# SimonMacLean/NeRF-or-nothing

Measured on AMD Instinct MI355X. Metric: train rays/sec (128 samples/ray, 8×256 MLP) at 1/2/4/8 MI355X; PSNR vs ref, higher is better.
Workload: dtype f32; 1 GPU; BASELINE configs[1]: 1024-ray global batch x 128+128 samples, 8x256 MLP fwd/bwd + Adam; global_batch=1024, rays_per_gpu=1024, micro_batch=1024, parallelism=dp1, precision=f32

## Files before the change

nerf-or-nothing_amd/csrc/host/accelerated.cpp:

```cpp
#include "accelerated.h"

#include <algorithm>
#include <cmath>
#include <cstring>

#include "../kernels/common.h"
#include "../kernels/mlp_common.h"
#include "../kernels/mlp_h32.h"
#include "trace.h"

namespace AcceleratedNeRFUtils {

using nof::kBlk;

void KernelTimer::enable(uint32_t mask, hipStream_t st) {
  mask_ = mask;
  st_ = st;
  used_ = 0;
  recs_.clear();
  for (int i = 0; i < NOF_NUM_TIMERS; ++i) { tot_ms_[i] = 0.0f; tot_n_[i] = 0; }
}
void KernelTimer::fold() {
  if (!recs_.empty()) NOF_HIP(hipEventSynchronize(recs_.back().b));
  for (const Rec& r : recs_) {
// ... 553 lines not shown
  }
  if ((size_t)so > slab_cap_ || items.size() * 256 > bias_slabs_.n) {
    NOF_HIP(hipStreamSynchronize(st_));
    slab_cap_ = std::max((size_t)so, slab_cap_);
    slabs_.alloc(slab_cap_);
    bias_slabs_.alloc(std::max(items.size() * 256, bias_slabs_.n));
  }
  std::vector<nof::WgOut> outs;
  int max_elems = 0;
  for (const OutSpec& s : os) {
    nof::WgOut o;
    o.item0 = first_item[s.prob];
    o.nitems = 0;
    NOF_REQUIRE(nlev <= nof::kWgMaxLevels, "too many levels");
    o.nlev = nlev;
    for (int l = 0; l < nlev; ++l) {
      NOF_REQUIRE(first_item[s.prob + l] == o.item0 + o.nitems, "a problem's items are not contiguous");
      o.lev_items[l] = nitems[s.prob + l];
      o.nitems += nitems[s.prob + l];
    }
    o.row_off = s.row_off; o.nrows = s.nrows; o.col_off = s.col_off; o.ncols = s.ncols;
    o.dst = s.dst; o.ld = s.ld; o.dst_col = s.dst_col; o.bias_dst = s.bias; o.prob = s.prob;
    outs.push_back(o);
    max_elems = std::max(max_elems, nof::wgrad_reduce_threads(s.nrows, s.ncols, s.col_off));
  }
  Schedule& sc = sched_[key];
  sc.probs.alloc(P.size());
  sc.items.alloc(items.size());
  sc.item_ptr.alloc(item_ptr.size());
  sc.slab_off.alloc(slab_off.size());
  sc.outs.alloc(outs.size());
  NOF_HIP(hipMemcpy(sc.probs.p, P.data(), P.size() * sizeof(P[0]), hipMemcpyHostToDevice));
  NOF_HIP(hipMemcpy(sc.items.p, items.data(), items.size() * sizeof(items[0]), hipMemcpyHostToDevice));
  NOF_HIP(hipMemcpy(sc.item_ptr.p, item_ptr.data(), item_ptr.size() * sizeof(int), hipMemcpyHostToDevice));
  NOF_HIP(hipMemcpy(sc.slab_off.p, slab_off.data(), slab_off.size() * sizeof(int64_t), hipMemcpyHostToDevice));
  NOF_HIP(hipMemcpy(sc.outs.p, outs.data(), outs.size() * sizeof(outs[0]), hipMemcpyHostToDevice));
  sc.nouts = (int)outs.size();
  sc.max_elems = max_elems;
  sc.num_wg = nwg;
  sc.lv0 = lv0;
  return sc;
}

void AcceleratedMLP::run_wgrad(Schedule& sc, int accumulate) {
  tb(kTWgrad);
  if (precision_ != NOF_PRECISION_F32)
    NOF_HIP(nof::launch_wgrad_x3(sc.probs.p, sc.items.p, sc.item_ptr.p, sc.num_wg, sc.slab_off.p, slabs_.p,
                                 bias_slabs_.p, precision_, st_));
  else
    NOF_HIP(nof::launch_wgrad(sc.probs.p, sc.items.p, sc.item_ptr.p, sc.num_wg, sc.slab_off.p, slabs_.p,
                              bias_slabs_.p, st_));
  te(kTWgrad);
  tb(kTWgradReduce);
  NOF_HIP(nof::launch_wgrad_reduce(sc.outs.p, sc.nouts, sc.max_elems, sc.items.p, sc.probs.p, sc.slab_off.p,
                                   slabs_.p, bias_slabs_.p, accumulate,
                                   f16_pieces() ? amax_.p + sc.lv0 : nullptr, st_));
  te(kTWgradReduce);
}

nof::BwdArgs AcceleratedMLP::bwd_args(int level, const float* color_grad, const float* density_grad) {
  Level& L = lv_[level];
  nof::BwdArgs b{};
  b.M = L.M;
  b.split = precision_;
  b.dbias = cfg_.density_bias;
  b.rgb_scale = rgb_scale();
  if (f16_pieces()) {
    if ((amax_given_ >> level) & 1u) {
      amax_given_ &= ~(1u << level);
    } else {
      const bool cleared = (amax_cleared_ >> level) & 1u;
      amax_cleared_ &= ~(1u << level);
      NOF_HIP(nof::launch_delta_amax(density_grad, color_grad, L.M, amax_.p + level, st_, numeric_.p, cleared));
    }
    b.amax = amax_.p + level;
  }
  b.dsigma = density_grad; b.drgb = color_grad; b.zhead = L.zhead.p;
  b.masks = L.masks.p;
  b.wimg_b = wimg_b_.p;
  b.delta = L.delta.p; b.delta9x = L.delta9x.p;
  return b;
}

void AcceleratedMLP::run_backward(int level, const float* color_grad, const float* density_grad) {
  const nof::BwdArgs b = bwd_args(level, color_grad, density_grad);
  tb(kTMlpBwd);
  NOF_HIP(nof::launch_mlp_bwd(b, st_));
  te(kTMlpBwd);
}

void AcceleratedMLP::run_backward2(int level, const float* const* color_grads, const float* const* density_grads) {
  nof::BwdArgs b = bwd_args(level, color_grads[0], density_grads[0]);
  const nof::BwdArgs b1 = bwd_args(level + 1, color_grads[1], density_grads[1]);
  b.M1 = b1.M; b.dsigma1 = b1.dsigma; b.drgb1 = b1.drgb; b.zhead1 = b1.zhead; b.amax1 = b1.amax;
  b.masks1 = b1.masks; b.delta1 = b1.delta; b.delta9x1 = b1.delta9x;
  tb(kTMlpBwd);
  NOF_HIP(nof::launch_mlp_bwd(b, st_));
  te(kTMlpBwd);
}

float* const* AcceleratedMLP::wgrad_levels(int lv0, int lv1, int accumulate, bool buckets) {
  if (!buckets) {
    run_wgrad(schedule(lv0, lv1), accumulate);
  } else {
    for (int bk = 0; bk < kBuckets; ++bk) {
      run_wgrad(schedule(lv0, lv1, bk), accumulate);
      int64_t off[2], cnt[2];
      const int ns = bucket_spans(bk, off, cnt);
      TraceRange hr("nof:gradient_bucket_hook");
      hook_(hook_user_, bk, ns, off, cnt);
    }
  }
  return grad_views_.data();
}

float* const* AcceleratedMLP::get_gradient(const float* color_grad, const float* density_grad, int level,
                                           uint32_t flags) {
  NOF_REQUIRE(level >= 0 && level < (int)lv_.size(), "level out of range");
  Level& L = lv_[level];
  NOF_REQUIRE(L.M > 0, "get_gradient before get_output for this level");
  NOF_REQUIRE(color_grad && density_grad, "null output gradients");
  NOF_REQUIRE((flags & ~(uint32_t)(NOF_GRAD_ACCUMULATE | NOF_GRAD_PUBLISH)) == 0, "unknown gradient flags");
  const bool buckets = (flags & NOF_GRAD_PUBLISH) && hook_;
  if (generic_) {
    gen_backward(level, color_grad, density_grad, (level > 0 || (flags & NOF_GRAD_ACCUMULATE)) ? 1 : 0);
    return gen_publish(buckets);
  }
  if (!buckets) (void)schedule(level, level + 1);
  else
    for (int b = 0; b < kBuckets; ++b) (void)schedule(level, level + 1, b);
  run_backward(level, color_grad, density_grad);
  return wgrad_levels(level, level + 1, (level > 0 || (flags & NOF_GRAD_ACCUMULATE)) ? 1 : 0, buckets);
}

float* const* AcceleratedMLP::get_gradient_levels(const float* const* color_grads, const float* const* density_grads,
                                                  uint32_t flags) {
  const int nl = (int)lv_.size();
  NOF_REQUIRE(color_grads && density_grads, "null output gradients");
  for (int l = 0; l < nl; ++l) {
    NOF_REQUIRE(lv_[l].M > 0, "get_gradient before get_output for a level");
    NOF_REQUIRE(color_grads[l] && density_grads[l], "null output gradients");
  }
  NOF_REQUIRE((flags & ~(uint32_t)(NOF_GRAD_ACCUMULATE | NOF_GRAD_PUBLISH)) == 0, "unknown gradient flags");
  const bool buckets = (flags & NOF_GRAD_PUBLISH) && hook_;
  if (generic_) {
    for (int l = 0; l < nl; ++l)
      gen_backward(l, color_grads[l], density_grads[l], (l > 0 || (flags & NOF_GRAD_ACCUMULATE)) ? 1 : 0);
    return gen_publish(buckets);
  }
  if (!buckets) (void)schedule(0, nl);
  else
    for (int b = 0; b < kBuckets; ++b) (void)schedule(0, nl, b);
  int l = 0;
  if (precision_ == NOF_PRECISION_F16)
    for (; l + 1 < nl; l += 2) run_backward2(l, color_grads + l, density_grads + l);
  for (; l < nl; ++l) run_backward(l, color_grads[l], density_grads[l]);
  return wgrad_levels(0, nl, (flags & NOF_GRAD_ACCUMULATE) ? 1 : 0, buckets);
}

static nof::GemmSrc gsrc(const float* p, int64_t si, int64_t sk, int idiv = 1) {
  nof::GemmSrc s;
  s.p = p; s.si = si; s.sk = sk; s.idiv = idiv;
  return s;
}

bool AcceleratedMLP::gen_product(nof::GemmArgs a, int ksplit, bool ws, bool f32) {
  int v;
  if (ksplit == 1) {
    a.kchunk = (a.K1 + a.K2 + 15) / 16 * 16;
    a.slab_stride = 0;
  }
  if (ws && !f16_products() && (!a.G || a.mask_in)) {
    nof::GemmArgs w = a;
    w.G = nullptr;
    if (nof::gemm_ws_fits(w)) {
      NOF_HIP(nof::launch_gemm_ws(w, st_, &v));
      tally(v);
      return true;
    }
  }
  NOF_REQUIRE(a.G || !a.mask_in, "a ReLU-bit mask needs the weight-stationary kernel");
  a.mask_in = nullptr;
  a.mask_out = nullptr;
  if (f16_products() && !f32) {
    NOF_HIP(nof::launch_gemm_h(a, ksplit, st_, &v));
    tally_h(v);
  } else {
    NOF_HIP(nof::launch_gemm(a, ksplit, st_, &v));
    tally(v);
  }
  return false;
}

void AcceleratedMLP::gen_split(int nout, int ncols, int M, int* ksplit, int* kchunk) {
  const int tiles = ((nout + 63) / 64) * ((ncols + 63) / 64);
  int ks = std::max(1, std::min((1024 + tiles - 1) / tiles, M / 64));
  const int kc = ((M + ks - 1) / ks + 15) / 16 * 16;
  *kchunk = kc;
  *ksplit = (M + kc - 1) / kc;
}

void AcceleratedMLP::gen_alloc() {
  const int NL = cfg_.num_levels;
  lv_.resize(NL);
  gl_.resize(NL);
  for (int l = 0; l < NL; ++l) {
    Level& L = lv_[l];
    GenLevel& G = gl_[l];
    L.cap = cfg_.max_rays * cfg_.num_samples[l];
    const size_t M = L.cap;
    G.mean.alloc(3 * M); G.cov.alloc(3 * M);
    G.enc_pos.alloc(M * gP_);
    G.enc_dir.alloc((size_t)cfg_.max_rays * gVd_);
    G.h.alloc((size_t)gD_ * M * gW_);
    G.hc.alloc((size_t)gDc_ * M * gWc_);
    G.z.alloc(4 * M);
    G.mbits.alloc((size_t)(gD_ + gDc_) * M * 4);
    G.mb_ok.assign(gD_ + gDc_, 0);
    L.sigma.alloc(M);
    L.rgb.alloc(3 * M);
    max_M_ = std::max(max_M_, L.cap);
  }
  const size_t Wm = std::max(gW_, gWc_);
  gd0_.alloc((size_t)max_M_ * Wm);
  gd1_.alloc((size_t)max_M_ * Wm);
  gdz_.alloc((size_t)max_M_ * 4);
  gray_.alloc((size_t)cfg_.max_rays * gWc_);
  if (cross_) denc_alloc(1);
  if (f16_products()) {
    amax_.alloc(NL);
    NOF_HIP(hipMemset(amax_.p, 0, NL * sizeof(uint32_t)));
  }
  size_t slab = 0;
  for (int l = 0; l < NL; ++l) {
    Level& L = lv_[l];
    size_t need = 0;
    wg_need_ = &need;
    L.M = L.cap; L.n = cfg_.max_rays; L.S = cfg_.num_samples[l];
    gen_backward(l, nullptr, nullptr, 0);
    L.M = L.n = L.S = 0;
    slab = std::max(slab, need);
  }
  wg_need_ = nullptr;
  gslab_.alloc(std::max<size_t>(slab, 1));
}

void AcceleratedMLP::denc_alloc(int first_level) {
  size_t Mx = 0;
  for (int l = first_level; l < (int)lv_.size(); ++l) Mx = std::max(Mx, (size_t)lv_[l].cap);
  int contrib = 1;
  for (int l = 1; l < gD_; ++l) contrib += l % gskip_ == 0 ? 1 : 0;
  const size_t parts = contrib > 2 ? (size_t)((contrib + 1) / 2) : 0;
  if (gd2_.n >= Mx * gW_ && gdenc_.n >= Mx * gP_ && gdenc_part_.n >= parts * Mx * gP_) return;
  if (gd2_.p) NOF_HIP(hipStreamSynchronize(st_));
  gd2_.alloc(Mx * gW_);
  gdenc_.alloc(Mx * gP_);
  if (parts) gdenc_part_.alloc(parts * Mx * gP_);
}

void AcceleratedMLP::set_ray_grad(bool on) {
  if (on) {
    if (!generic_)
      throw Error(NOF_ERR_UNSUPPORTED,
                  "ray gradients need the any-shape path: the fused 8x256 kernels produce no gradient of the encoded "
                  "input (use NOF_PRECISION_F16_PRODUCTS, or NOF_PRECISION_F32 with stop_level_grad = 0)");
    denc_alloc(0);
    if (!gddir_.p) {
      gddir_.alloc((size_t)cfg_.max_rays * gVd_);
      rg_o_.alloc(3 * (size_t)cfg_.max_rays);
      rg_d_.alloc(3 * (size_t)cfg_.max_rays);
    }
  }
  ray_grad_ = on;
  rg_job_ = RayGradJob();
}

void AcceleratedMLP::gen_wgrad(float* dst, int64_t ld, const float* dz, int64_t ldz, int nout, nof::GemmSrc x,
                               int ncols, int M, int accumulate, float* bias_dst, const uint32_t* scale) {
  int ks, kc;
  gen_split(nout, ncols, M, &ks, &kc);
  const size_t need = (size_t)ks * nout * (ncols + 1);
  if (wg_need_) {
    *wg_need_ += need;
    return;
  }
  NOF_REQUIRE(wg_off_ + need <= gslab_.n, "split-K slabs too small");
  float* slab = gslab_.p + wg_off_;
  wg_off_ += need;
  nof::GemmArgs a;
  a.M = nout; a.N = ncols; a.K1 = M;
  a.A1 = gsrc(dz, 1, ldz);
  a.B1 = x;
  a.C = slab; a.ci = ncols; a.cj = 1;
  a.kchunk = kc; a.slab_stride = (int64_t)nout * ncols;
  float* bias_part = slab + (size_t)ks * nout * ncols;
  if (bias_dst) a.rowsum = bias_part;
  if (scale) { a.scale_amax = scale; a.scale_src = 1; }
  gen_product(a, ks, false, !scale);
  wg_jobs_.push_back({slab, dst, a.slab_stride, ld, nout, ncols, ncols, ks, accumulate});
  if (bias_dst) wg_jobs_.push_back({bias_part, bias_dst, nout, nout, 1, nout, nout, ks, accumulate});
}

void AcceleratedMLP::gen_forward(int level, const float* ep, const float* ed) {
  Level& L = lv_[level];
  GenLevel& G = gl_[level];
  const int M = L.M, S = L.S, D = gD_, W = gW_, Dc = gDc_, Wc = gWc_, P = gP_, Vd = gVd_, lr = D + 1 + Dc;
  G.ep = ep; G.ed = ed;
// ... 668 lines not shown
```

nerf-or-nothing_amd/csrc/kernels/mlp16.h:

```cpp
#pragma once
#include "mlp_common.h"

namespace nof {

constexpr int kMlp16Threads = 512;
constexpr int kIpe16Floats = 6 * 64 * 4;

__device__ __forceinline__ f32x4 mfma16(float a, float b, f32x4 c) {
  return __builtin_amdgcn_mfma_f32_16x16x4f32(a, b, c, 0, 0, 0);
}

__device__ __forceinline__ void slice16_dma_step(const float* __restrict__ src, float* dst, int tid, int i) {
  const int wave = tid >> 6;
  const __amdgpu_buffer_rsrc_t rsrc =
      __builtin_amdgcn_make_buffer_rsrc(const_cast<float*>(src), (short)0, 0x7fffffff, 0x00020000);
  __builtin_amdgcn_raw_ptr_buffer_load_lds(rsrc, (lptr_t)(dst + (kMlp16Threads * i + 64 * wave) * 4), 16, tid * 16,
                                           i * kMlp16Threads * 16, 0, 0);
}
__device__ __forceinline__ void slice16_dma(const float* __restrict__ src, float* dst, int tid) {
#pragma unroll
  for (int i = 0; i < 4; ++i) slice16_dma_step(src, dst, tid, i);
}

template <int P> constexpr int ring16_slots() { return P == 0 ? 4 : 3; }
template <int P> constexpr int ring16_floats() { return ring16_slots<P>() * kSliceFloats; }
__device__ __forceinline__ void ring16_prologue(const float* __restrict__ img, float* lds, int tid) {
  slice16_dma(img, lds, tid);
  slice16_dma(img + kSliceFloats, lds + kSliceFloats, tid);
}

__device__ __forceinline__ constexpr int feat16(int t, int g, int r) { return 16 * t + 4 * g + r; }

constexpr int kStoreNT = 2;
struct BlkStore16 {
  static constexpr bool kHalf = false;
  uint32_t voff[4];
  __device__ __forceinline__ BlkStore16(int lane, int half) {
    const int g = lane >> 4, s = 16 * half + (lane & 15);
#pragma unroll
    for (int r = 0; r < 4; ++r)
      voff[r] = 512u * g + ((((s >> 2) ^ (4 * (g & 1) + r)) << 4) | ((s & 3) << 2));
  }
  __device__ __forceinline__ void store(__amdgpu_buffer_rsrc_t blk, int t, int r, float v) const {
    __builtin_amdgcn_raw_buffer_store_b32(__float_as_uint(v), blk, (int)voff[r], 2048 * t + 128 * r, kStoreNT);
  }
};
__device__ __forceinline__ __amdgpu_buffer_rsrc_t blk_rsrc(float* blk) {
  return __builtin_amdgcn_make_buffer_rsrc(blk, (short)0, 0x7fffffff, 0x00020000);
}

template <bool kNT>
struct BlkStore16H {
  static constexpr bool kHalf = true;
  uint32_t voff;
  uint32_t voff2;
  uint32_t sel;
  __device__ __forceinline__ BlkStore16H(int lane, int half) {
    const int g = lane >> 4, j = lane & 15;
    voff = 256u * g + ((((2 * half + (j >> 3)) ^ g) << 4) | ((j & 7) << 1));
    voff2 = 256u * g + 64u * (j & 1) + ((((2 * half + (j >> 3)) ^ g) << 4) | ((j & 6) << 1));
    sel = (j & 1) ? 0x03020706u : 0x05040100u;
  }
  __device__ __forceinline__ void store_pairs(__amdgpu_buffer_rsrc_t blk, int t, uint32_t p01, uint32_t p23) const {
    const uint32_t q01 = (uint32_t)__builtin_amdgcn_mov_dpp((int)p01, 0xB1, 0xF, 0xF, false);
    const uint32_t q23 = (uint32_t)__builtin_amdgcn_mov_dpp((int)p23, 0xB1, 0xF, 0xF, false);
    __builtin_amdgcn_raw_buffer_store_b32(__builtin_amdgcn_perm(q01, p01, sel), blk, (int)voff2, 1024 * t,
                                          kNT ? kStoreNT : 0);
    __builtin_amdgcn_raw_buffer_store_b32(__builtin_amdgcn_perm(q23, p23, sel), blk, (int)voff2 + 128, 1024 * t,
                                          kNT ? kStoreNT : 0);
  }
  __device__ __forceinline__ void store(__amdgpu_buffer_rsrc_t blk, int t, int r, float v) const {
    store_h(blk, t, r, (_Float16)v);
  }
  __device__ __forceinline__ void store_h(__amdgpu_buffer_rsrc_t blk, int t, int r, _Float16 h) const {
    __builtin_amdgcn_raw_buffer_store_b16(__builtin_bit_cast(unsigned short, h), blk, (int)voff + 64 * r, 1024 * t,
                                          kNT ? kStoreNT : 0);
  }
};
template <int P, bool kBwd> struct Store16 { typedef BlkStore16 T; typedef float E; };
template <bool kBwd> struct Store16<2, kBwd> { typedef BlkStore16H<true> T; typedef _Float16 E; };
template <class E>
__device__ __forceinline__ __amdgpu_buffer_rsrc_t blk_rsrc_t(E* blk) {
  return __builtin_amdgcn_make_buffer_rsrc(blk, (short)0, 0x7fffffff, 0x00020000);
}

__device__ __forceinline__ uint2* mask16_ptr(uint32_t* masks, int blk, int slot, int half, int lane) {
  return reinterpret_cast<uint2*>(mask_ptr(masks, blk, slot) + half * 128) + lane;
}
__device__ __forceinline__ bool mask16_bit(const uint2& m, int t, int r) {
  return ((t >> 3 ? m.y : m.x) >> (31 - ((t & 7) * 4 + r))) & 1u;
}
__device__ __forceinline__ float mask16_apply(const uint2& m, int t, int r, float v) {
  const uint32_t w = t >> 3 ? m.y : m.x;
  uint32_t all;
  asm("v_bfe_i32 %0, %1, %2, 1" : "=v"(all) : "v"(w), "n"(31 - ((t & 7) * 4 + r)));
  return __uint_as_float(__float_as_uint(v) & all);
}

__device__ __forceinline__ float relu_bit(float z, uint32_t& mw) {
  const int h = max(__float_as_int(z), 0);
  asm volatile("v_cmp_lt_i32 vcc, 0, %1\n\tv_addc_co_u32 %0, vcc, %0, %0, vcc" : "+v"(mw) : "v"(h) : "vcc");
  return __int_as_float(h);
}

__device__ __forceinline__ void split4h(const float (&x)[4], uint32_t& hi01, uint32_t& hi23, uint32_t& lo01,
                                        uint32_t& lo23) {
  typedef _Float16 h2 __attribute__((ext_vector_type(2)));
  typedef float f2 __attribute__((ext_vector_type(2)));
  hi01 = __builtin_bit_cast(uint32_t, __builtin_convertvector((f2{x[0], x[1]}), h2));
  hi23 = __builtin_bit_cast(uint32_t, __builtin_convertvector((f2{x[2], x[3]}), h2));
  float r[4];
  asm("v_fma_mix_f32 %0, %1, 1.0, -%2 op_sel_hi:[0,0,1]" : "=v"(r[0]) : "v"(x[0]), "v"(hi01));
  asm("v_fma_mix_f32 %0, %1, 1.0, -%2 op_sel:[0,0,1] op_sel_hi:[0,0,1]" : "=v"(r[1]) : "v"(x[1]), "v"(hi01));
  asm("v_fma_mix_f32 %0, %1, 1.0, -%2 op_sel_hi:[0,0,1]" : "=v"(r[2]) : "v"(x[2]), "v"(hi23));
  asm("v_fma_mix_f32 %0, %1, 1.0, -%2 op_sel:[0,0,1] op_sel_hi:[0,0,1]" : "=v"(r[3]) : "v"(x[3]), "v"(hi23));
  lo01 = __builtin_bit_cast(uint32_t, __builtin_convertvector((f2{r[0], r[1]}), h2));
  lo23 = __builtin_bit_cast(uint32_t, __builtin_convertvector((f2{r[2], r[3]}), h2));
}

template <bool kSplit, bool kStore, class ST>
__device__ __forceinline__ void put_tile(float (&bin)[16][4], int t, const float (&v)[4], const ST& bst,
                                         __amdgpu_buffer_rsrc_t blk) {
  if constexpr (kSplit) {
    uint32_t hi01, hi23, lo01, lo23;
    split4h(v, hi01, hi23, lo01, lo23);
    const int row = t & ~1, c = 2 * (t & 1);
    bin[row][c] = __uint_as_float(hi01);
    bin[row][c + 1] = __uint_as_float(hi23);
    bin[row + 1][c] = __uint_as_float(lo01);
    bin[row + 1][c + 1] = __uint_as_float(lo23);
    if constexpr (kStore) {
      if constexpr (ST::kHalf) {
        bst.store_pairs(blk, t, hi01, hi23);
      } else {
#pragma unroll
        for (int r = 0; r < 4; ++r) bst.store(blk, t, r, v[r]);
      }
    }
  } else {
#pragma unroll
    for (int r = 0; r < 4; ++r) {
      bin[t][r] = v[r];
      if constexpr (kStore) bst.store(blk, t, r, v[r]);
    }
  }
}

struct NoEpi16 {
  static constexpr int kVmPerPart = 0;
  __device__ __forceinline__ void operator()(int) {}
};

template <int NT_B, int NT_I, int OT, int kSlots, class Epi>
__device__ __forceinline__ void mlp_layer16(const float (&bin)[16][4], const float* ipe, f32x4 (&acc)[16],
                                            float* lds, int& cur, const float*& wsrc, bool last_in_schedule, int tid,
                                            int lane, Epi& epi, const float* cinit) {
  static_assert(OT % 2 == 0 && OT <= 16, "row tiles come in pairs");
  constexpr int NG = OT;
  constexpr int kEpiGroup1 = 4;
  constexpr int kEpiGroup2 = (NG / 2 + 4 < NG) ? NG / 2 + 4 : NG - 1;
  const int g = lane >> 4;
  const int row = lane & 15;
  const int swz = (row >> 1) & 7;
#pragma unroll
  for (int t = 0; t < NT_B + NT_I; ++t) {
    const bool dma = !(last_in_schedule && t + 2 >= NT_B + NT_I);
    const int nxt2 = kSlots == 4 ? ((cur + 2) & 3) : (cur == 0 ? 2 : cur - 1);
    const float* W = lds + cur * kSliceFloats + row * 32;
    auto aread = [&](int q, int which) {
      const int tt = q / (OT / 2), p = q % (OT / 2);
      return *reinterpret_cast<const f32x4*>(W + (2 * p + which) * 16 * 32 + (((4 * tt + g) ^ swz) << 2));
    };
    f32x4 a0 = aread(0, 0), a1 = aread(0, 1);
    auto cread = [&](int p, int which) { return *reinterpret_cast<const f32x4*>(cinit + 16 * (2 * p + which)); };
    f32x4 c0 = {}, c1 = {};
    if (t == 0 && cinit) { c0 = cread(0, 0); c1 = cread(0, 1); }
#pragma unroll
    for (int q = 0; q < NG; ++q) {
      const int tt = q / (OT / 2), p = q % (OT / 2);
      f32x4 b4;
      if (t < NT_B) {
        const int tb = (t < NT_B) ? 2 * t + tt : 0;
        b4[0] = bin[tb][0]; b4[1] = bin[tb][1]; b4[2] = bin[tb][2]; b4[3] = bin[tb][3];
      } else {
        const int ti = (t >= NT_B) ? 2 * (t - NT_B) + tt : 0;
        if constexpr (kSlots == 4) {
          b4[0] = ipe[4 * ti]; b4[1] = ipe[4 * ti + 1]; b4[2] = ipe[4 * ti + 2]; b4[3] = ipe[4 * ti + 3];
        } else b4 = *reinterpret_cast<const f32x4*>(ipe + (ti * 64 + lane) * 4);
      }
      asm volatile("" ::"v"(a0), "v"(a1), "v"(c0), "v"(c1));
      f32x4 n0 = a0, n1 = a1, m0 = c0, m1 = c1;
      if (q + 1 < NG) {
        n0 = aread(q + 1, 0);
        n1 = aread(q + 1, 1);
      }
      if (t == 0 && cinit && q + 1 < OT / 2) { m0 = cread(q + 1, 0); m1 = cread(q + 1, 1); }
      if (dma && q < 4) slice16_dma_step(wsrc + 2 * kSliceFloats, lds + nxt2 * kSliceFloats, tid, q);
      __builtin_amdgcn_sched_barrier(0);
      const bool first = t == 0 && tt == 0;
#pragma unroll
      for (int r = 0; r < 4; ++r) {
        acc[2 * p] = mfma16(a0[r], b4[r], (first && r == 0) ? c0 : acc[2 * p]);
        acc[2 * p + 1] = mfma16(a1[r], b4[r], (first && r == 0) ? c1 : acc[2 * p + 1]);
      }
      if (t + 1 < NT_B && q == kEpiGroup1) epi(2 * t + 2);
      if (t + 1 < NT_B && q == kEpiGroup2) epi(2 * t + 3);
      __builtin_amdgcn_sched_barrier(0);
      a0 = n0;
      a1 = n1;
      c0 = m0;
      c1 = m1;
    }
    if constexpr (kSlots == 4) {
      if (cur & 1) slice_barrier(t + 1 < NT_B ? 2 * Epi::kVmPerPart : 0);
      cur = (cur + 1) & 3;
    } else {
      slice_barrier((dma ? 4 : 0) + (t + 1 < NT_B ? 2 * Epi::kVmPerPart : 0));
      cur = cur == 2 ? 0 : cur + 1;
    }
    wsrc += kSliceFloats;
  }
}
template <int NT_B, int NT_I, int OT, class Epi>
__device__ __forceinline__ void mlp_layer16h(const float (&bin)[16][4], const float* ipe_lds, f32x4 (&acc)[16],
                                             float* lds, int& cur, const float*& wsrc, bool last_in_schedule, int tid,
                                             int lane, Epi& epi, const float* cinit) {
  typedef SplitMode<2> SM;
  static_assert(OT % 2 == 0 && OT <= 16, "row tiles come in pairs");
  constexpr int kPieces = 2;
  constexpr int kPP0 = 0;
  constexpr int kDmaSteps = 4;
  constexpr int kSlots = ring16_slots<2>();
  constexpr int NG = OT / 2;
  constexpr int kE1 = NG > 4 ? 4 : NG - 1;
  constexpr int kE2 = NG > 6 ? 6 : NG - 1;
#pragma unroll
  for (int t = 0; t < NT_B + NT_I; ++t) {
    const bool dma = !(last_in_schedule && t + 2 >= NT_B + NT_I);
    const int nxt2 = kSlots == 4 ? ((cur + 2) & 3) : (cur == 0 ? 2 : cur - 1);
    const f16x8* W = reinterpret_cast<const f16x8*>(lds + cur * kSliceFloats) + lane;
    Frag<2> b;
    float v[8];
    if (t < NT_B) {
      const int tb = t < NT_B ? 2 * t : 0;
      const f32x4 hi = {bin[tb][0], bin[tb][1], bin[tb][2], bin[tb][3]};
      const f32x4 lo = {bin[tb + 1][0], bin[tb + 1][1], bin[tb + 1][2], bin[tb + 1][3]};
      b.p[0] = __builtin_bit_cast(f16x8, hi);
      b.p[1] = __builtin_bit_cast(f16x8, lo);
    } else {
      const int ti = t >= NT_B ? 2 * (t - NT_B) : 0;
      if constexpr (kSlots == 4) {
#pragma unroll
        for (int i = 0; i < 8; ++i) v[i] = ipe_lds[4 * ti + i];
      } else {
        const f32x4 u0 = *reinterpret_cast<const f32x4*>(ipe_lds + (ti * 64 + lane) * 4);
        const f32x4 u1 = *reinterpret_cast<const f32x4*>(ipe_lds + ((ti + 1) * 64 + lane) * 4);
#pragma unroll
        for (int i = 0; i < 4; ++i) { v[i] = u0[i]; v[4 + i] = u1[i]; }
      }
      split8<2>(v, b);
    }
    Frag<2> a0, a1;
#pragma unroll
    for (int p = 0; p < kPieces; ++p) { a0.p[p] = W[(16 * p) * 64]; a1.p[p] = W[(16 * p + 1) * 64]; }
    auto cread = [&](int rt) { return *reinterpret_cast<const f32x4*>(cinit + 16 * rt); };
    f32x4 c0 = {}, c1 = {};
    if (t == 0 && cinit) { c0 = cread(0); c1 = cread(1); }
#pragma unroll
    for (int q = 0; q < NG; ++q) {
      if constexpr (kPieces == 2) asm volatile("" ::"v"(a0.p[0]), "v"(a0.p[1]), "v"(a1.p[0]), "v"(a1.p[1]), "v"(c0), "v"(c1));
      else asm volatile("" ::"v"(a0.p[0]), "v"(a1.p[0]), "v"(c0), "v"(c1));
      Frag<2> n0 = a0, n1 = a1;
      f32x4 m0 = c0, m1 = c1;
      if (t == 0 && cinit && q + 1 < NG) { m0 = cread(2 * q + 2); m1 = cread(2 * q + 3); }
      if (q + 1 < NG) {
#pragma unroll
        for (int p = 0; p < kPieces; ++p) {
          n0.p[p] = W[(16 * p + 2 * q + 2) * 64];
          n1.p[p] = W[(16 * p + 2 * q + 3) * 64];
        }
      }
      if (dma && q < kDmaSteps) slice16_dma_step(wsrc + 2 * kSliceFloats, lds + nxt2 * kSliceFloats, tid, q);
      __builtin_amdgcn_sched_barrier(0);
      const bool first = t == 0;
#pragma unroll
      for (int pp = kPP0; pp < SM::NPROD; ++pp) {
        acc[2 * q] = SM::mfma16(a0.p[SM::pa(pp)], b.p[SM::pb(pp)], (first && pp == kPP0) ? c0 : acc[2 * q]);
        acc[2 * q + 1] = SM::mfma16(a1.p[SM::pa(pp)], b.p[SM::pb(pp)], (first && pp == kPP0) ? c1 : acc[2 * q + 1]);
      }
      if (t + 1 < NT_B && q == kE1) epi(2 * t + 2);
      if (t + 1 < NT_B && q == kE2) epi(2 * t + 3);
      __builtin_amdgcn_sched_barrier(0);
      a0 = n0;
      a1 = n1;
      c0 = m0;
      c1 = m1;
    }
    if constexpr (kSlots == 4) {
      if (cur & 1) slice_barrier(t + 1 < NT_B ? 2 * Epi::kVmPerPart : 0);
      cur = (cur + 1) & 3;
    } else {
      slice_barrier((dma ? kDmaSteps : 0) + (t + 1 < NT_B ? 2 * Epi::kVmPerPart : 0));
      cur = cur == 2 ? 0 : cur + 1;
    }
    wsrc += kSliceFloats;
  }
}

template <int P, int NT_B, int NT_I, int OT, class Epi>
__device__ __forceinline__ void layer16(const float (&bin)[16][4], const float* ipe_lds, f32x4 (&acc)[16], float* lds,
                                        int& cur, const float*& wsrc, bool last_in_schedule, int tid, int lane,
                                        Epi& epi, const float* cinit = nullptr) {
  if constexpr (P == 2 || P == 3)
    mlp_layer16h<NT_B, NT_I, OT>(bin, ipe_lds, acc, lds, cur, wsrc, last_in_schedule, tid, lane, epi, cinit);
  else
    mlp_layer16<NT_B, NT_I, OT, ring16_slots<P>()>(bin, ipe_lds, acc, lds, cur, wsrc, last_in_schedule, tid, lane,
                                                   epi, cinit);
}
template <int P, int NT_B, int NT_I, int OT>
__device__ __forceinline__ void layer16(const float (&bin)[16][4], const float* ipe_lds, f32x4 (&acc)[16], float* lds,
                                        int& cur, const float*& wsrc, bool last_in_schedule, int tid, int lane,
                                        const float* cinit = nullptr) {
  NoEpi16 none;
  layer16<P, NT_B, NT_I, OT>(bin, ipe_lds, acc, lds, cur, wsrc, last_in_schedule, tid, lane, none, cinit);
}

}
```

nerf-or-nothing_amd/csrc/kernels/mlp_bwd16.hip:

```cpp
#include "common.h"
#include "launch.h"
#include "mlp16.h"

namespace nof {


template <bool kDensity, class ST, bool kSplit = false>
struct BwdEpi16 {
  static constexpr int kVmPerPart = 4;
  const f32x4 (&acc)[16];
  float (&bin)[16][4];
  const ST& bst;
  const int g;
  const float* w8;
  float dzs;
  __amdgpu_buffer_rsrc_t dst_blk;
  uint2 mk;
  f32x4 wnext;

  __device__ __forceinline__ BwdEpi16(const f32x4 (&acc_)[16], float (&bin_)[16][4], const ST& bst_, int lane)
      : acc(acc_), bin(bin_), bst(bst_), g(lane >> 4) {}
  template <class E>
  __device__ __forceinline__ void begin(const uint2* mask, E* dst_blk_, const float* w8_ = nullptr, float dzs_ = 0.0f) {
    mk = *mask;
    dst_blk = blk_rsrc_t(dst_blk_);
    if constexpr (kDensity) {
      w8 = w8_ + 4 * g;
      dzs = dzs_;
      wnext = *reinterpret_cast<const f32x4*>(w8);
    }
  }
  __device__ __forceinline__ void operator()(int t) {
    f32x4 w4;
    if constexpr (kDensity) {
      w4 = wnext;
      if (t + 1 < 16) wnext = *reinterpret_cast<const f32x4*>(w8 + 16 * (t + 1));
    }
    float v[4];
#pragma unroll
    for (int r = 0; r < 4; ++r) {
      v[r] = acc[t][r];
      if constexpr (kDensity) v[r] = __builtin_fmaf(w4[r], dzs, v[r]);
      v[r] = mask16_apply(mk, t, r, v[r]);
    }
    put_tile<kSplit, true>(bin, t, v, bst, dst_blk);
  }
  __device__ __forceinline__ void tile01() {
    (*this)(0);
    (*this)(1);
  }
};

template <int P>
__global__ __launch_bounds__(kMlp16Threads, 1) void k_mlp_bwd16(BwdArgs a) {
  typedef typename Store16<P, true>::T ST;
  typedef typename Store16<P, true>::E AE;
  __shared__ __attribute__((aligned(16))) float lds[ring16_floats<P>() + 256];
  float* w8_lds = lds + ring16_floats<P>();
  const int tid = threadIdx.x, lane = tid & 63, g = lane >> 4, j = lane & 15;
  const int wave = __builtin_amdgcn_readfirstlane(tid >> 6);
  const int half = wave & 1;
  const ST bst(lane, half);
  const int nblk = a.M / kBlk;
  const int blk_raw = blockIdx.x * 4 + (wave >> 1);
  const int blk = blk_raw < nblk ? blk_raw : nblk - 1;
  const int m = blk * kBlk + 16 * half + j;
  NOF_DCHECK(a.M % kBlk == 0 && blk >= 0 && blk < nblk, kChkMlpBlock);
  const float* tail = a.wimg_b + (size_t)kBwdSlices * kSliceFloats;
  const size_t layer_stride = (size_t)nblk * kWidth * kBlk;
  uint32_t* masks = const_cast<uint32_t*>(a.masks);

  ring16_prologue(a.wimg_b, lds, tid);

  const f32x4 zh = reinterpret_cast<const f32x4*>(a.zhead)[m];
  float dzs = a.dsigma[m] * sigmoid_f(zh[0] + a.dbias);
  float dzc[3];
#pragma unroll
  for (int c = 0; c < 3; ++c) {
    const float s = sigmoid_f(zh[1 + c]);
    dzc[c] = a.drgb[(size_t)m * 3 + c] * (s * (1.0f - s)) * a.rgb_scale;
  }
  if constexpr (P >= 2) {
    const float sc = delta_scale(a.amax, false);
    dzs *= sc;
#pragma unroll
    for (int c = 0; c < 3; ++c) dzc[c] *= sc;
  }
  const __amdgpu_buffer_rsrc_t d9 = blk_rsrc_t(reinterpret_cast<AE*>(a.delta9x) + (size_t)blk * kD9F * kBlk);
#pragma unroll
  for (int r = 0; r < 4; ++r) bst.store(d9, 8, r, g == 0 ? (r == 0 ? dzs : dzc[r - 1]) : 0.0f);
  float bin[16][4];
  {
    const uint2 mk = *mask16_ptr(masks, blk, 8, half, lane);
    const float* w10 = tail + kBwdTailW10;
#pragma unroll
    for (int t = 0; t < 8; ++t) {
      const int fb = 16 * t + 4 * g;
      const f32x4 wa = *reinterpret_cast<const f32x4*>(w10 + fb);
      const f32x4 wb = *reinterpret_cast<const f32x4*>(w10 + 128 + fb);
      const f32x4 wc = *reinterpret_cast<const f32x4*>(w10 + 256 + fb);
      float v[4];
#pragma unroll
      for (int r = 0; r < 4; ++r)
        v[r] = mask16_apply(mk, t, r, __builtin_fmaf(wc[r], dzc[2], __builtin_fmaf(wb[r], dzc[1], wa[r] * dzc[0])));
      put_tile<P >= 2, true>(bin, t, v, bst, d9);
    }
  }
  if (tid < 64) reinterpret_cast<f32x4*>(w8_lds)[tid] = reinterpret_cast<const f32x4*>(tail + kBwdTailW8)[tid];
  __syncthreads();

  int cur = 0;
  const float* wsrc = a.wimg_b;
  f32x4 accA[16], accB[16];
  AE* delta_blk = reinterpret_cast<AE*>(a.delta) + (size_t)blk * kWidth * kBlk;
  BwdEpi16<true, ST, P >= 2> e7(accA, bin, bst, lane);
  e7.begin(mask16_ptr(masks, blk, 7, half, lane), delta_blk + 7 * layer_stride, w8_lds, dzs);
  layer16<P, 4, 0, 16>(bin, nullptr, accA, lds, cur, wsrc, false, tid, lane);
  e7.tile01();
  BwdEpi16<false, ST, P >= 2> ea(accA, bin, bst, lane), eb(accB, bin, bst, lane);
  eb.begin(mask16_ptr(masks, blk, 6, half, lane), delta_blk + 6 * layer_stride);
  layer16<P, 8, 0, 16>(bin, nullptr, accB, lds, cur, wsrc, false, tid, lane, e7);
  eb.tile01();
  static_assert(kDepth == 8, "bwd pairing assumes 8 trunk layers");
  for (int l = kDepth - 2; l >= 2; l -= 2) {
    ea.begin(mask16_ptr(masks, blk, l - 1, half, lane), delta_blk + (l - 1) * layer_stride);
    layer16<P, 8, 0, 16>(bin, nullptr, accA, lds, cur, wsrc, false, tid, lane, eb);
    ea.tile01();
    eb.begin(mask16_ptr(masks, blk, l - 2, half, lane), delta_blk + (l - 2) * layer_stride);
    layer16<P, 8, 0, 16>(bin, nullptr, accB, lds, cur, wsrc, l == 2, tid, lane, ea);
    eb.tile01();
  }
#pragma unroll
  for (int t = 2; t < 16; ++t) eb(t);
}

hipError_t launch_mlp_bwd16(const BwdArgs& a, hipStream_t st) {
  const int nblk = a.M / kBlk;
  if (a.split == 2) hipLaunchKernelGGL(k_mlp_bwd16<2>, dim3((nblk + 3) / 4), dim3(kMlp16Threads), 0, st, a);
  else if (a.split == 3) hipLaunchKernelGGL(k_mlp_bwd16<3>, dim3((nblk + 3) / 4), dim3(kMlp16Threads), 0, st, a);
  else hipLaunchKernelGGL(k_mlp_bwd16<0>, dim3((nblk + 3) / 4), dim3(kMlp16Threads), 0, st, a);
  return hipGetLastError();
}

NOF_CHECK_UNIT(check_unit_mlp_bwd16)

}
```

Before: 163,700 rays/s.

## Make f32 MLP backward a persistent kernel spanning both levels with prefetch

The f32 backward MLP kernel becomes persistent: the grid is capped at the CU count and each block loops over block-groups from both levels, coarse and fine. While the last layer of the current group runs, it DMAs the next group's per-ray inputs and the first weight slices into LDS, which hides prologue latency and launch overhead. W10 and W8 are staged in LDS once per block. The host now uses the paired run_backward2 path for F32 too. In exchange the kernel uses more LDS and inline asm LDS reads, and it relies on the run_backward2 path setting M1 and the second-level pointers correctly.

```diff
diff --git a/nerf-or-nothing_amd/csrc/host/accelerated.cpp b/nerf-or-nothing_amd/csrc/host/accelerated.cpp
--- a/nerf-or-nothing_amd/csrc/host/accelerated.cpp
+++ b/nerf-or-nothing_amd/csrc/host/accelerated.cpp
@@ -729,7 +729,7 @@
   else
     for (int b = 0; b < kBuckets; ++b) (void)schedule(0, nl, b);
   int l = 0;
-  if (precision_ == NOF_PRECISION_F16)
+  if (precision_ == NOF_PRECISION_F16 || precision_ == NOF_PRECISION_F32)
     for (; l + 1 < nl; l += 2) run_backward2(l, color_grads + l, density_grads + l);
   for (; l < nl; ++l) run_backward(l, color_grads[l], density_grads[l]);
   return wgrad_levels(0, nl, (flags & NOF_GRAD_ACCUMULATE) ? 1 : 0, buckets);
diff --git a/nerf-or-nothing_amd/csrc/kernels/mlp16.h b/nerf-or-nothing_amd/csrc/kernels/mlp16.h
--- a/nerf-or-nothing_amd/csrc/kernels/mlp16.h
+++ b/nerf-or-nothing_amd/csrc/kernels/mlp16.h
@@ -154,7 +154,7 @@
 template <int NT_B, int NT_I, int OT, int kSlots, class Epi>
 __device__ __forceinline__ void mlp_layer16(const float (&bin)[16][4], const float* ipe, f32x4 (&acc)[16],
                                             float* lds, int& cur, const float*& wsrc, bool last_in_schedule, int tid,
-                                            int lane, Epi& epi, const float* cinit) {
+                                            int lane, Epi& epi, const float* cinit, const float* wrap_src) {
   static_assert(OT % 2 == 0 && OT <= 16, "row tiles come in pairs");
   constexpr int NG = OT;
   constexpr int kEpiGroup1 = 4;
@@ -164,7 +164,10 @@
   const int swz = (row >> 1) & 7;
 #pragma unroll
   for (int t = 0; t < NT_B + NT_I; ++t) {
-    const bool dma = !(last_in_schedule && t + 2 >= NT_B + NT_I);
+    const bool past = last_in_schedule && t + 2 >= NT_B + NT_I;
+    const float* src2 = !past ? wsrc + 2 * kSliceFloats
+                              : (wrap_src ? wrap_src + (t + 2 - (NT_B + NT_I)) * kSliceFloats : nullptr);
+    const bool dma = src2 != nullptr;
     const int nxt2 = kSlots == 4 ? ((cur + 2) & 3) : (cur == 0 ? 2 : cur - 1);
     const float* W = lds + cur * kSliceFloats + row * 32;
     auto aread = [&](int q, int which) {
@@ -195,7 +198,7 @@
         n1 = aread(q + 1, 1);
       }
       if (t == 0 && cinit && q + 1 < OT / 2) { m0 = cread(q + 1, 0); m1 = cread(q + 1, 1); }
-      if (dma && q < 4) slice16_dma_step(wsrc + 2 * kSliceFloats, lds + nxt2 * kSliceFloats, tid, q);
+      if (dma && q < 4) slice16_dma_step(src2, lds + nxt2 * kSliceFloats, tid, q);
       __builtin_amdgcn_sched_barrier(0);
       const bool first = t == 0 && tt == 0;
 #pragma unroll
@@ -310,12 +313,12 @@
 template <int P, int NT_B, int NT_I, int OT, class Epi>
 __device__ __forceinline__ void layer16(const float (&bin)[16][4], const float* ipe_lds, f32x4 (&acc)[16], float* lds,
                                         int& cur, const float*& wsrc, bool last_in_schedule, int tid, int lane,
-                                        Epi& epi, const float* cinit = nullptr) {
+                                        Epi& epi, const float* cinit = nullptr, const float* wrap_src = nullptr) {
   if constexpr (P == 2 || P == 3)
     mlp_layer16h<NT_B, NT_I, OT>(bin, ipe_lds, acc, lds, cur, wsrc, last_in_schedule, tid, lane, epi, cinit);
   else
     mlp_layer16<NT_B, NT_I, OT, ring16_slots<P>()>(bin, ipe_lds, acc, lds, cur, wsrc, last_in_schedule, tid, lane,
-                                                   epi, cinit);
+                                                   epi, cinit, wrap_src);
 }
 template <int P, int NT_B, int NT_I, int OT>
 __device__ __forceinline__ void layer16(const float (&bin)[16][4], const float* ipe_lds, f32x4 (&acc)[16], float* lds,
diff --git a/nerf-or-nothing_amd/csrc/kernels/mlp_bwd16.hip b/nerf-or-nothing_amd/csrc/kernels/mlp_bwd16.hip
--- a/nerf-or-nothing_amd/csrc/kernels/mlp_bwd16.hip
+++ b/nerf-or-nothing_amd/csrc/kernels/mlp_bwd16.hip
@@ -1,3 +1,5 @@
+#include <algorithm>
+
 #include "common.h"
 #include "launch.h"
 #include "mlp16.h"
@@ -51,34 +53,134 @@
   }
 };
 
+__device__ __forceinline__ uint32_t lane_id_opaque() {
+  uint32_t id;
+  asm volatile("v_mbcnt_lo_u32_b32 %0, -1, 0\n\tv_mbcnt_hi_u32_b32 %0, -1, %0" : "=v"(id));
+  return id;
+}
+__device__ __forceinline__ int opaque_vgpr(int v) {
+  asm volatile("" : "+v"(v));
+  return v;
+}
+__device__ __forceinline__ void bwd16_read_inputs(uint32_t base, uint32_t lane, uint32_t j, uint2& mk, f32x4& zh,
+                                                  float (&dr)[3], float& ds) {
+  typedef uint32_t u32x2 __attribute__((ext_vector_type(2)));
+  u32x2 mkv;
+  asm volatile(
+      "ds_read_b64 %0, %6\n\tds_read_b128 %1, %7 offset:512\n\tds_read_b32 %2, %8 offset:768\n\t"
+      "ds_read_b32 %3, %8 offset:772\n\tds_read_b32 %4, %8 offset:776\n\tds_read_b32 %5, %9 offset:960\n\t"
+      "s_waitcnt lgkmcnt(0)"
+      : "=&v"(mkv), "=&v"(zh), "=&v"(dr[0]), "=&v"(dr[1]), "=&v"(dr[2]), "=&v"(ds)
+      : "v"(base + 8u * lane), "v"(base + 16u * j), "v"(base + 12u * j), "v"(base + 4u * j)
+      : "memory");
+  mk = {mkv[0], mkv[1]};
+}
+__device__ __forceinline__ void lds_dma16(const void* p, float* dst, uint32_t voff) {
+  __builtin_amdgcn_raw_ptr_buffer_load_lds(
+      __builtin_amdgcn_make_buffer_rsrc(const_cast<void*>(p), (short)0, 0x7fffffff, 0x00020000), (lptr_t)dst, 16,
+      voff, 0, 0, 0);
+}
+__device__ __forceinline__ void lds_dma4(const void* p, float* dst, uint32_t voff) {
+  __builtin_amdgcn_raw_ptr_buffer_load_lds(
+      __builtin_amdgcn_make_buffer_rsrc(const_cast<void*>(p), (short)0, 0x7fffffff, 0x00020000), (lptr_t)dst, 4,
+      voff, 0, 0, 0);
+}
+__device__ __forceinline__ uint32_t lds_addr(const float* p) {
+  return (uint32_t)(uintptr_t)(__attribute__((address_space(3))) const void*)p;
+}
+__device__ __forceinline__ void wait_vm0() { asm volatile("s_waitcnt vmcnt(0)" ::: "memory"); }
+
 template <int P>
 __global__ __launch_bounds__(kMlp16Threads, 1) void k_mlp_bwd16(BwdArgs a) {
   typedef typename Store16<P, true>::T ST;
   typedef typename Store16<P, true>::E AE;
-  __shared__ __attribute__((aligned(16))) float lds[ring16_floats<P>() + 256];
-  float* w8_lds = lds + ring16_floats<P>();
-  const int tid = threadIdx.x, lane = tid & 63, g = lane >> 4, j = lane & 15;
-  const int wave = __builtin_amdgcn_readfirstlane(tid >> 6);
+  constexpr bool kPersist = P == 0;
+  constexpr int kW8 = ring16_floats<P>(), kW10 = kW8 + 256, kIn = kW10 + 3 * 128, kInFloats = 256;
+  __shared__ __attribute__((aligned(16))) float lds[kPersist ? kIn + 8 * kInFloats : kW8 + 256];
+  float* w8_lds = lds + kW8;
+  const int tid0 = threadIdx.x;
+  const int wave = __builtin_amdgcn_readfirstlane(tid0 >> 6);
   const int half = wave & 1;
+  const float* tail = a.wimg_b + (size_t)kBwdSlices * kSliceFloats;
+  const int nblk0 = a.M / kBlk, nblk1 = kPersist ? a.M1 / kBlk : 0;
+  const int ng0 = (nblk0 + 3) / 4, ngroups = ng0 + (nblk1 + 3) / 4;
+  NOF_DCHECK(a.M % kBlk == 0 && (!kPersist || a.M1 % kBlk == 0) && (int)blockIdx.x < ngroups, kChkMlpBlock);
+  struct GrpLv {
+    int nblk, blk;
+    const float *dsigma, *drgb, *zhead;
+    uint32_t* masks;
+    float *delta, *delta9x;
+  };
+  auto grp = [&](int gg) {
+    GrpLv v;
+    const bool second = kPersist && gg >= ng0;
+    v.nblk = second ? nblk1 : nblk0;
+    v.blk = min((second ? gg - ng0 : gg) * 4 + (wave >> 1), v.nblk - 1);
+    v.dsigma = second ? a.dsigma1 : a.dsigma;
+    v.drgb = second ? a.drgb1 : a.drgb;
+    v.zhead = second ? a.zhead1 : a.zhead;
+    v.masks = const_cast<uint32_t*>(second ? a.masks1 : a.masks);
+    v.delta = second ? a.delta1 : a.delta;
+    v.delta9x = second ? a.delta9x1 : a.delta9x;
+    return v;
+  };
+  float* const in_slot = lds + kIn + wave * kInFloats;
+  auto in_dma = [&](int gg) {
+    const GrpLv v = grp(gg);
+    const int m0 = v.blk * kBlk + 16 * half;
+    const uint32_t id = lane_id_opaque();
+    if (id < 32) lds_dma16(mask16_ptr(v.masks, v.blk, 8, half, 0), in_slot, id * 16);
+    if (id < 16) {
+      lds_dma16(v.zhead + (size_t)m0 * 4, in_slot + 128, id * 16);
+      lds_dma4(v.dsigma + m0, in_slot + 240, id * 4);
+    }
+    if (id < 12) lds_dma16(v.drgb + (size_t)m0 * 3, in_slot + 192, id * 16);
+  };
+
+  ring16_prologue(a.wimg_b, lds, tid0);
+  if constexpr (kPersist) {
+    in_dma(blockIdx.x);
+    if (tid0 >= 64 && tid0 < 160)
+      reinterpret_cast<f32x4*>(lds + kW10)[tid0 - 64] = reinterpret_cast<const f32x4*>(tail + kBwdTailW10)[tid0 - 64];
+  }
+  if (tid0 < 64) reinterpret_cast<f32x4*>(w8_lds)[tid0] = reinterpret_cast<const f32x4*>(tail + kBwdTailW8)[tid0];
+  if constexpr (kPersist) {
+    wait_vm0();
+    __syncthreads();
+  }
+
+  int gi = blockIdx.x;
+  do {
+  int cur = 0;
+  const int tid = kPersist ? opaque_vgpr(tid0) : tid0;
+  const int lane = tid & 63, g = lane >> 4, j = lane & 15;
   const ST bst(lane, half);
-  const int nblk = a.M / kBlk;
-  const int blk_raw = blockIdx.x * 4 + (wave >> 1);
-  const int blk = blk_raw < nblk ? blk_raw : nblk - 1;
-  const int m = blk * kBlk + 16 * half + j;
-  NOF_DCHECK(a.M % kBlk == 0 && blk >= 0 && blk < nblk, kChkMlpBlock);
-  const float* tail = a.wimg_b + (size_t)kBwdSlices * kSliceFloats;
+  const GrpLv lv = grp(gi);
+  const int nblk = lv.nblk, blk = lv.blk;
+  NOF_DCHECK(blk >= 0 && blk < nblk, kChkMlpBlock);
   const size_t layer_stride = (size_t)nblk * kWidth * kBlk;
-  uint32_t* masks = const_cast<uint32_t*>(a.masks);
-
-  ring16_prologue(a.wimg_b, lds, tid);
-
-  const f32x4 zh = reinterpret_cast<const f32x4*>(a.zhead)[m];
-  float dzs = a.dsigma[m] * sigmoid_f(zh[0] + a.dbias);
+  uint32_t* masks = lv.masks;
+  const bool has_next = kPersist && gi + (int)gridDim.x < ngroups;
+
+  f32x4 zh;
+  float ds_m, dr[3];
+  uint2 mk9;
+  if constexpr (kPersist) {
+    bwd16_read_inputs(lds_addr(in_slot), lane, j, mk9, zh, dr, ds_m);
+  } else {
+    const int m = blk * kBlk + 16 * half + j;
+    zh = reinterpret_cast<const f32x4*>(lv.zhead)[m];
+    ds_m = lv.dsigma[m];
+#pragma unroll
+    for (int c = 0; c < 3; ++c) dr[c] = lv.drgb[(size_t)m * 3 + c];
+    mk9 = *mask16_ptr(masks, blk, 8, half, lane);
+  }
+  float dzs = ds_m * sigmoid_f(zh[0] + a.dbias);
   float dzc[3];
 #pragma unroll
   for (int c = 0; c < 3; ++c) {
     const float s = sigmoid_f(zh[1 + c]);
-    dzc[c] = a.drgb[(size_t)m * 3 + c] * (s * (1.0f - s)) * a.rgb_scale;
+    dzc[c] = dr[c] * (s * (1.0f - s)) * a.rgb_scale;
   }
   if constexpr (P >= 2) {
     const float sc = delta_scale(a.amax, false);
@@ -86,13 +188,13 @@
 #pragma unroll
     for (int c = 0; c < 3; ++c) dzc[c] *= sc;
   }
-  const __amdgpu_buffer_rsrc_t d9 = blk_rsrc_t(reinterpret_cast<AE*>(a.delta9x) + (size_t)blk * kD9F * kBlk);
+  const __amdgpu_buffer_rsrc_t d9 = blk_rsrc_t(reinterpret_cast<AE*>(lv.delta9x) + (size_t)blk * kD9F * kBlk);
 #pragma unroll
   for (int r = 0; r < 4; ++r) bst.store(d9, 8, r, g == 0 ? (r == 0 ? dzs : dzc[r - 1]) : 0.0f);
   float bin[16][4];
   {
-    const uint2 mk = *mask16_ptr(masks, blk, 8, half, lane);
-    const float* w10 = tail + kBwdTailW10;
+    const uint2 mk = mk9;
+    const float* w10 = kPersist ? lds + kW10 : tail + kBwdTailW10;
 #pragma unroll
     for (int t = 0; t < 8; ++t) {
       const int fb = 16 * t + 4 * g;
@@ -106,13 +208,11 @@
       put_tile<P >= 2, true>(bin, t, v, bst, d9);
     }
   }
-  if (tid < 64) reinterpret_cast<f32x4*>(w8_lds)[tid] = reinterpret_cast<const f32x4*>(tail + kBwdTailW8)[tid];
-  __syncthreads();
-
-  int cur = 0;
+  if constexpr (!kPersist) __syncthreads();
+
   const float* wsrc = a.wimg_b;
   f32x4 accA[16], accB[16];
-  AE* delta_blk = reinterpret_cast<AE*>(a.delta) + (size_t)blk * kWidth * kBlk;
+  AE* delta_blk = reinterpret_cast<AE*>(lv.delta) + (size_t)blk * kWidth * kBlk;
   BwdEpi16<true, ST, P >= 2> e7(accA, bin, bst, lane);
   e7.begin(mask16_ptr(masks, blk, 7, half, lane), delta_blk + 7 * layer_stride, w8_lds, dzs);
   layer16<P, 4, 0, 16>(bin, nullptr, accA, lds, cur, wsrc, false, tid, lane);
@@ -122,23 +222,35 @@
   layer16<P, 8, 0, 16>(bin, nullptr, accB, lds, cur, wsrc, false, tid, lane, e7);
   eb.tile01();
   static_assert(kDepth == 8, "bwd pairing assumes 8 trunk layers");
+  static_assert(kBwdSlices % 4 == 0, "a group ends in the ring slot it started in");
   for (int l = kDepth - 2; l >= 2; l -= 2) {
     ea.begin(mask16_ptr(masks, blk, l - 1, half, lane), delta_blk + (l - 1) * layer_stride);
     layer16<P, 8, 0, 16>(bin, nullptr, accA, lds, cur, wsrc, false, tid, lane, eb);
     ea.tile01();
     eb.begin(mask16_ptr(masks, blk, l - 2, half, lane), delta_blk + (l - 2) * layer_stride);
-    layer16<P, 8, 0, 16>(bin, nullptr, accB, lds, cur, wsrc, l == 2, tid, lane, ea);
+    if (l == 2 && has_next) in_dma(gi + gridDim.x);
+    layer16<P, 8, 0, 16>(bin, nullptr, accB, lds, cur, wsrc, l == 2, tid, lane, ea, nullptr,
+                         has_next ? a.wimg_b : nullptr);
     eb.tile01();
   }
 #pragma unroll
   for (int t = 2; t < 16; ++t) eb(t);
+  gi += gridDim.x;
+  } while (kPersist && gi < ngroups);
 }
 
 hipError_t launch_mlp_bwd16(const BwdArgs& a, hipStream_t st) {
   const int nblk = a.M / kBlk;
-  if (a.split == 2) hipLaunchKernelGGL(k_mlp_bwd16<2>, dim3((nblk + 3) / 4), dim3(kMlp16Threads), 0, st, a);
-  else if (a.split == 3) hipLaunchKernelGGL(k_mlp_bwd16<3>, dim3((nblk + 3) / 4), dim3(kMlp16Threads), 0, st, a);
-  else hipLaunchKernelGGL(k_mlp_bwd16<0>, dim3((nblk + 3) / 4), dim3(kMlp16Threads), 0, st, a);
+  if (a.split == 2 || a.split == 3) {
+    if (a.M1 != 0) return hipErrorInvalidValue;
+    if (a.split == 2) hipLaunchKernelGGL(k_mlp_bwd16<2>, dim3((nblk + 3) / 4), dim3(kMlp16Threads), 0, st, a);
+    else hipLaunchKernelGGL(k_mlp_bwd16<3>, dim3((nblk + 3) / 4), dim3(kMlp16Threads), 0, st, a);
+    return hipGetLastError();
+  }
+  if (a.M1 < 0 || a.M1 % kBlk != 0) return hipErrorInvalidValue;
+  const int ngroups = (nblk + 3) / 4 + (a.M1 / kBlk + 3) / 4;
+  const dim3 grid(std::min(ngroups, device_cus()));
+  hipLaunchKernelGGL(k_mlp_bwd16<0>, grid, dim3(kMlp16Threads), 0, st, a);
   return hipGetLastError();
 }
 
```

Result: no change. 164,500 rays/s (median of 4 runs) (+0.4%).
